# saiakarsh193/GenVox

Hardware: NVIDIA B200
Metric: Tacotron2 train mel-frames/s (higher is better)
Workload: dtype bf16

## Files before the change

genvox_b200/csrc/gvx_fused_bwd.cuh:

```cuda
#pragma once
#include <cooperative_groups.h>
#include <cuda_bf16.h>

#include "gvx_fused_fwd.cuh"

namespace gvx {

constexpr int FB_THREADS = 512;
constexpr int FB_NCOL = 48;
constexpr int FB_KSLAB = 16;
constexpr int FB_WSLAB_BYTES = FB_NCOL * 128;
constexpr int FB_RING = 8;
constexpr int FB_WLD_LD = 136;
constexpr int FB_QBYTES = FB_KSLAB * PC_CHUNK_BYTES;
constexpr int FB_PLD = 68;
constexpr int FB_DWQ = 5;

struct FbGeom {
    int RS, NH, NHP, nblk, NDS, nmt;
    __host__ __device__ FbGeom(int N, int RS_) {
        RS = RS_;
        NH = (((N + RS - 1) / RS) + 7) & ~7;
        NHP = (NH + 15) & ~15;
        nblk = NH / 8;
        NDS = NH + 40;
        nmt = NHP / 16;
    }
};

struct FbShared {
    uint64_t full[FB_RING], empty[FB_RING], tmem_full, wbar, thbar, xb[4];
    uint32_t tmem_slot;
    volatile int dead;
};

struct FbSmem {
    int ring, ths, dhqp, dqs, pdw, wsm, pin, cpart, dconvT, wlc, wldh, dctx, ctx32, w, de, dal, dwc, dcumc, v, xch, sh, total;
    __host__ __device__ FbSmem(int N, int RS) {
        const FbGeom g(N, RS);
        int o = 0;
        auto take = [&](int bytes) { int r = o; o += (bytes + 127) & ~127; return r; };
        ring = 0;
        ths = take(g.NHP * AF_D * 2);
        dqs = take(PC_ROWS * AF_D * 2);
        dhqp = take(4 * PC_ROWS * 8 * 4);
        pdw = take(16 * g.NHP * 4);
        o = o > FB_RING * PC_CHUNK_BYTES ? ((o + 1023) & ~1023) : FB_RING * PC_CHUNK_BYTES;
        wsm = take(FB_KSLAB * FB_WSLAB_BYTES);
        pin = take(4 * 12 * FB_PLD * 4);
        cpart = take(16 * 2 * g.NHP * 4);
        dconvT = take(AF_F * g.NDS * 4);
        wlc = take(AF_F * 2 * AF_KS * 4);
        wldh = take(AF_F * FB_WLD_LD * 2);
        dctx = take(FA_E * 4);
        ctx32 = take(FA_E * 4);
        w = take(g.NHP * 4);
        de = take(g.NHP * 4);
        dal = take(g.NHP * 4);
        dwc = take(g.NHP * 4);
        dcumc = take(g.NHP * 4);
        v = take(AF_D * 4);
        xch = take(64);
        sh = take((int)sizeof(FbShared));
        total = o + 1024;
    }
};

struct FbArgs {
    const __nv_bfloat16 *Wimg;
    uint8_t *gimg;
    const __nv_bfloat16 *WqB;
    const float *gates_stash;
    const float *c_stash;
    const float *dxdall;
    const float *dhc;
    int Kp, H;
    const float *d_align;
    const float *align;
    const float *ctx32;
    const __nv_bfloat16 *th;
    const __nv_bfloat16 *memb;
    const float *wlc, *wldT, *v;
    const int64_t *lengths;
    __nv_bfloat16 *dg_rm;
    __nv_bfloat16 *dq_rm;
    float *de_out;
    uint16_t *dconv_out;
    float *dctx_out;
    unsigned long long *dctxx;
    unsigned long long *dqx;
    unsigned *bar;
    int *err;
    DropCfg drop;
    int row_offset, B, N, T, RS;
    long long *dbg;
};

__device__ __forceinline__ void fb_gstamp(long long *dbg, int cta, int i, int k) {
    if (dbg && i == 20) dbg[32 * 1024 + cta * 16 + k] = fa_globaltimer();
}
__device__ __forceinline__ void fb_bar_w14() { asm volatile("bar.sync 2, 448;" ::: "memory"); }
__device__ __forceinline__ void st_async_f32(uint32_t caddr, float v, uint32_t cmbar) {
    asm volatile("st.async.weak.shared::cluster.mbarrier::complete_tx::bytes.f32 [%0], %1, [%2];" ::"r"(caddr), "f"(v), "r"(cmbar) : "memory");
}
__device__ __forceinline__ void st_async_f32x2(uint32_t caddr, float v0, float v1, uint32_t cmbar) {
    asm volatile("st.async.weak.shared::cluster.mbarrier::complete_tx::bytes.v2.f32 [%0], {%1, %2}, [%3];" ::"r"(caddr), "f"(v0), "f"(v1), "r"(cmbar)
                 : "memory");
}
__device__ __forceinline__ bool fb_wait_warp(uint64_t *bar, uint32_t parity, volatile int *dead, int *err, int code) {
    int ok = 1;
    if ((threadIdx.x & 31) == 0) ok = fa_wait_cluster(bar, parity, dead, err, code) ? 1 : 0;
    ok = __shfl_sync(0xffffffffu, ok, 0);
    if (ok) {
        while (!mbar_try_wait_cluster(bar, parity)) {}
    }
    return ok != 0;
}
__device__ __forceinline__ float4 fb_lstm_bwd_point(float dh_dropped, float mult, float4 ga, float c_prev, float c_new, float dc_in,
                                                    float &dc_prev) {
    const float dh = dh_dropped * mult;
    const float tc = tanh_fast(c_new);
    const float d_o = dh * tc;
    const float dc = dc_in + dh * ga.w * (1.f - tc * tc);
    const float d_i = dc * ga.z, d_g = dc * ga.x, d_f = dc * c_prev;
    dc_prev = dc * ga.y;
    return make_float4(d_i * ga.x * (1.f - ga.x), d_f * ga.y * (1.f - ga.y), d_g * (1.f - ga.z * ga.z), d_o * ga.w * (1.f - ga.w));
}

__global__ void __cluster_dims__(4, 1, 1) __launch_bounds__(FB_THREADS, 1) k_att_chain_bwd(const FbArgs a) {
    namespace cg = cooperative_groups;
    cg::cluster_group cluster = cg::this_cluster();
    extern __shared__ uint8_t smem_raw[];
    uint8_t *smem = smem_raw + ((1024u - (smem_u32(smem_raw) & 1023u)) & 1023u);
    const int N = a.N, T = a.T, B = a.B, RS = a.RS;
    const FbGeom G(N, RS);
    const FbSmem L(N, RS);
    uint8_t *ring = smem + L.ring, *wsm = smem + L.wsm, *ths = smem + L.ths;
    float *pin = (float *)(smem + L.pin), *cpart = (float *)(smem + L.cpart), *pdw = (float *)(smem + L.pdw);
    uint8_t *dqs = smem + L.dqs;
    float *dconvT = (float *)(smem + L.dconvT), *wlc = (float *)(smem + L.wlc);
    __nv_bfloat16 *wldh = (__nv_bfloat16 *)(smem + L.wldh);
    float *dctx = (float *)(smem + L.dctx), *ctx32 = (float *)(smem + L.ctx32);
    float *ws = (float *)(smem + L.w), *des = (float *)(smem + L.de), *dals = (float *)(smem + L.dal);
    float *dwc = (float *)(smem + L.dwc), *dcumc = (float *)(smem + L.dcumc), *vs = (float *)(smem + L.v);
    float *dhqp = (float *)(smem + L.dhqp);
    float *xch = (float *)(smem + L.xch);
    FbShared *sh = (FbShared *)(smem + L.sh);

    const int tid = threadIdx.x, wid = tid >> 5, lane = tid & 31, j = blockIdx.x;
    const int g4 = lane >> 2, tig = lane & 3;
    const int r = (int)cluster.block_rank(), c = j >> 2;
    const int row = RS == 2 ? 2 * c + (r >> 1) : c;
    const int prt = RS == 2 ? (r & 1) : r;
    const int gbase = RS == 2 ? (r & ~1) : 0;
    const bool rvalid = row < B;
    const int rowc = rvalid ? row : B - 1;
    const int len = a.lengths ? (int)a.lengths[rowc] : N;
    const int n_lo = prt * G.NH;
    const int n_own = rvalid ? max(0, min(N, n_lo + G.NH) - n_lo) : 0;
    const int own_len = max(0, min(len, n_lo + n_own) - n_lo);
    const bool th_live = n_own > 0;
    const bool has_left = prt > 0, has_right = prt < RS - 1;
    const int uk = tid & 7, ub = tid >> 3, uu = 8 * j + uk;
    const int ck = tid & 3, cb = (tid >> 2) & 63;
    const bool uvalid = ub < B;

    if (tid == 0) {
        for (int s = 0; s < FB_RING; ++s) { mbar_init(sh->full + s, 1); mbar_init(sh->empty + s, 1); }
        mbar_init(&sh->tmem_full, 1);
        mbar_init(&sh->wbar, 1);
        mbar_init(&sh->thbar, 1);
        for (int k = 0; k < 4; ++k) mbar_init(sh->xb + k, 1);
        sh->dead = 0;
        asm volatile("fence.mbarrier_init.release.cluster;" ::: "memory");
        asm volatile("fence.proxy.async.shared::cta;" ::: "memory");
    }
    if (wid == 0) {
        asm volatile("tcgen05.alloc.cta_group::1.sync.aligned.shared::cta.b32 [%0], %1;" ::"r"(smem_u32(&sh->tmem_slot)), "n"(64) : "memory");
        asm volatile("tcgen05.relinquish_alloc_permit.cta_group::1.sync.aligned;" ::: "memory");
    }
    for (int i = tid; i < AF_F * 2 * AF_KS; i += FB_THREADS) wlc[i] = a.wlc[i];
    for (int i = tid; i < AF_F * AF_D; i += FB_THREADS) wldh[(i >> 7) * FB_WLD_LD + (i & 127)] = __float2bfloat16(a.wldT[i]);
    if (tid < AF_D) vs[tid] = a.v[tid];
    for (int i = tid; i < AF_F * G.NDS; i += FB_THREADS) dconvT[i] = 0.f;
    for (int i = tid; i < G.NHP * AF_D / 2; i += FB_THREADS) reinterpret_cast<uint32_t *>(ths)[i] = 0u;
    for (int i = tid; i < G.NHP; i += FB_THREADS) { ws[i] = 0.f; des[i] = 0.f; dals[i] = 0.f; dwc[i] = 0.f; dcumc[i] = 0.f; }
    if (tid < 16) xch[tid] = 0.f;
    tc_fence_before();
    __syncthreads();
    tc_fence_after();
    const uint32_t tmem_base = sh->tmem_slot;
    if (tid == 0) {
        asm volatile("fence.proxy.async.shared::cta;" ::: "memory");
        mbar_expect_tx(&sh->wbar, FB_KSLAB * FB_WSLAB_BYTES);
        const uint8_t *wsrc = (const uint8_t *)a.Wimg + (size_t)j * FB_KSLAB * FB_WSLAB_BYTES;
        for (uint32_t off = 0; off < FB_KSLAB * FB_WSLAB_BYTES; off += 16384) tma_bulk_g2s(wsm + off, wsrc + off, 16384, &sh->wbar);
        if (th_live) {
            mbar_expect_tx(&sh->thbar, (uint32_t)n_own * AF_D * 2);
            tma_bulk_g2s(ths, a.th + (((size_t)(T - 1) * B + row) * N + n_lo) * AF_D, (uint32_t)n_own * AF_D * 2, &sh->thbar);
        }
    }
    const int qm = wid & 3, kq = wid >> 2;
    uint32_t wqf[2][2];
#pragma unroll
    for (int s = 0; s < 2; ++s)
#pragma unroll
        for (int hh = 0; hh < 2; ++hh) {
            const int d0 = 16 * (2 * kq + s) + 2 * tig + 8 * hh;
            const __nv_bfloat16 lo = a.WqB[(size_t)d0 * FA_A + 8 * j + g4], hi = a.WqB[(size_t)(d0 + 1) * FA_A + 8 * j + g4];
            wqf[s][hh] = (uint32_t)__bfloat16_as_ushort(lo) | ((uint32_t)__bfloat16_as_ushort(hi) << 16);
        }
    const uint32_t my_xch = smem_u32(xch), my_xb0 = smem_u32(sh->xb + 0), my_xb3 = smem_u32(sh->xb + 3), my_pin = smem_u32(pin);
    const uint32_t halo_bytes = (uint32_t)(min(AF_PAD, G.NH) * AF_F * 4) * (uint32_t)((has_left ? 1 : 0) + (has_right ? 1 : 0));
    const uint32_t my_dqs = smem_u32(dqs), my_xb1 = smem_u32(sh->xb + 1);
    const uint32_t nbl_dconv = mapa_u32(smem_u32(dconvT), (uint32_t)(gbase + max(prt - 1, 0)));
    const uint32_t nbr_dconv = mapa_u32(smem_u32(dconvT), (uint32_t)(gbase + min(prt + 1, RS - 1)));
    const uint32_t nbl_xb2 = mapa_u32(smem_u32(sh->xb + 2), (uint32_t)(gbase + max(prt - 1, 0)));
    const uint32_t nbr_xb2 = mapa_u32(smem_u32(sh->xb + 2), (uint32_t)(gbase + min(prt + 1, RS - 1)));

    DropCfg drop = a.drop;
    if (drop.kptr) { drop.k0 = drop.kptr[0]; drop.k1 = drop.kptr[1]; drop.kptr = nullptr; }
    float dc = 0.f, rec = 0.f;
    float c_new = uvalid ? a.c_stash[((size_t)T * B + ub) * FA_A + uu] : 0.f;
    const int quarter = j >> 5;
    const int kk0 = 4 * uu - 1024 * quarter;
    const size_t gimg_off = (size_t)quarter * FB_QBYTES + (size_t)(kk0 >> 6) * PC_CHUNK_BYTES + ub * 128 +
                            ((((kk0 & 63) >> 3) ^ (ub & 7)) << 4) + (kk0 & 7) * 2;
    unsigned *bq_own = a.bar + 16 * quarter + ((j & 31) >> 1);
    const unsigned *bq_need = a.bar + 16 * r;
    const size_t AE = FA_A + FA_E;

    if (tid < FA_E) {
        dctx[tid] = rvalid ? a.dhc[((size_t)(T - 1) * B + row) * a.Kp + a.H + tid] + a.dxdall[((size_t)(T - 1) * B + row) * AE + FA_A + tid] : 0.f;
        ctx32[tid] = rvalid ? a.ctx32[((size_t)(T - 1) * B + row) * FA_E + tid] : 0.f;
    }
    if (tid < G.NHP) {
        ws[tid] = tid < n_own ? a.align[((size_t)row * T + (T - 1)) * N + n_lo + tid] : 0.f;
        dals[tid] = (a.d_align && tid < n_own) ? a.d_align[((size_t)row * T + (T - 1)) * N + n_lo + tid] : 0.f;
    }
    if (wid == 0 && a.d_align && rvalid) {
        const float *al = a.align + ((size_t)row * T + (T - 1)) * N, *dal = a.d_align + ((size_t)row * T + (T - 1)) * N;
        for (int q = 0; q < RS; ++q) {
            const int q_lo = q * G.NH, q_own = max(0, min(N, q_lo + G.NH) - q_lo), q_len = max(0, min(len, q_lo + q_own) - q_lo);
            float p = 0.f;
            for (int n = lane; n < q_len; n += 32) p = fmaf(al[q_lo + n], dal[q_lo + n], p);
            p = warp_sum(p);
            if (lane == 0) xch[q] = p;
        }
    }
    __syncthreads();
    cluster.sync();
    const bool okw = fa_wait_mbar(&sh->wbar, 0, &sh->dead, a.err, 51);

    float mult = uvalid ? drop_mult(drop, SITE_ATT, (uint32_t)(T - 1), (uint32_t)(ub + a.row_offset), (uint32_t)uu) : 1.f;
    const __nv_bfloat16 *memb_b = a.memb + ((size_t)rowc * N + n_lo) * FA_E;
    uint4 mv[FB_DWQ][2];
    auto load_mem = [&](int mt0) {
#pragma unroll
        for (int q = 0; q < FB_DWQ; ++q) {
#pragma unroll
            for (int h2 = 0; h2 < 2; ++h2) {
                const int n = 16 * (mt0 + q) + g4 + 8 * h2;
                mv[q][h2] = n < own_len ? __ldg(reinterpret_cast<const uint4 *>(memb_b + (size_t)n * FA_E + 32 * wid + 8 * tig)) : make_uint4(0u, 0u, 0u, 0u);
            }
        }
    };
    load_mem(0);
    for (int i = 0; i < T; ++i) {
        const int t = T - 1 - i;
        const uint32_t par = (uint32_t)i & 1u;
        if (tid == 0) { pc_stamp(a.dbg, j, i, 0); fb_gstamp(a.dbg, j, i, 0); }
        if (i > 0 && tid < FA_E) {
            const unsigned long long *src = a.dctxx + ((size_t)par * PC_ROWS + rowc) * FA_E + tid;
            unsigned long long wv = 0ull;
            fa_spin([&] { wv = ld_relaxed_u64(src); return (unsigned)(wv >> 32) == (unsigned)i; }, &sh->dead, a.err, 52);
            if (rvalid) dctx[tid] += __uint_as_float((unsigned)wv);
        }
        if (tid < FA_E && rvalid && prt == 0) a.dctx_out[((size_t)t * B + row) * FA_E + tid] = dctx[tid];
        if (i > 0) fb_wait_warp(sh->xb + 0, par ^ 1u, &sh->dead, a.err, 53);
        if (th_live) fb_wait_warp(&sh->thbar, par, &sh->dead, a.err, 54);
        __syncthreads();
        if (tid == 0) {
            pc_stamp(a.dbg, j, i, 1);
            fb_gstamp(a.dbg, j, i, 1);
            mbar_expect_tx(sh->xb + 1, (uint32_t)PC_ROWS * AF_D * 2);
            if (halo_bytes) mbar_expect_tx(sh->xb + 2, halo_bytes);
            if (i + 1 < T) {
                mbar_expect_tx(sh->xb + 0, (uint32_t)RS * 4);
                mbar_expect_tx(sh->xb + 3, 4u * 12u * PC_ROWS * 4u);
            }
        }
        {
            uint32_t bfr[4] = {0u, 0u, 0u, 0u};
            if (g4 < 2) {
                const float4 d0 = *reinterpret_cast<const float4 *>(dctx + 32 * wid + 8 * tig), d1 = *reinterpret_cast<const float4 *>(dctx + 32 * wid + 8 * tig + 4);
                float x[8] = {d0.x, d0.y, d0.z, d0.w, d1.x, d1.y, d1.z, d1.w};
                if (g4 == 1) {
#pragma unroll
                    for (int k = 0; k < 8; ++k) x[k] -= __bfloat162float(__float2bfloat16(x[k]));
                }
#pragma unroll
                for (int k = 0; k < 4; ++k) bfr[k] = pack_bf2(x[2 * k], x[2 * k + 1]);
            }
            for (int mt0 = 0; mt0 < G.nmt; mt0 += FB_DWQ) {
                if (mt0 > 0) load_mem(mt0);
#pragma unroll
                for (int q = 0; q < FB_DWQ; ++q) {
                    if (mt0 + q < G.nmt) {
                        float acc[4] = {0.f, 0.f, 0.f, 0.f};
                        mma_bf16_16816(acc, mv[q][0].x, mv[q][1].x, mv[q][0].y, mv[q][1].y, bfr[0], bfr[1]);
                        mma_bf16_16816(acc, mv[q][0].z, mv[q][1].z, mv[q][0].w, mv[q][1].w, bfr[2], bfr[3]);
                        if (tig == 0) {
                            pdw[wid * G.NHP + 16 * (mt0 + q) + g4] = acc[0] + acc[1];
                            pdw[wid * G.NHP + 16 * (mt0 + q) + g4 + 8] = acc[2] + acc[3];
                        }
                    }
                }
            }
        }
        __syncthreads();
        if (tid == 0) pc_stamp(a.dbg, j, i, 12);
        if (wid * 32 < G.NHP) {
            float dot = 0.f;
#pragma unroll
            for (int h2 = 0; h2 < 2; ++h2) {
                const float4 g0 = *reinterpret_cast<const float4 *>(dctx + lane * 8 + 256 * h2), g1 = *reinterpret_cast<const float4 *>(dctx + lane * 8 + 256 * h2 + 4);
                const float4 c0 = *reinterpret_cast<const float4 *>(ctx32 + lane * 8 + 256 * h2), c1 = *reinterpret_cast<const float4 *>(ctx32 + lane * 8 + 256 * h2 + 4);
                dot = fmaf(c0.x, g0.x, dot); dot = fmaf(c0.y, g0.y, dot); dot = fmaf(c0.z, g0.z, dot); dot = fmaf(c0.w, g0.w, dot);
                dot = fmaf(c1.x, g1.x, dot); dot = fmaf(c1.y, g1.y, dot); dot = fmaf(c1.z, g1.z, dot); dot = fmaf(c1.w, g1.w, dot);
            }
            dot = warp_sum(dot);
            for (int p = 0; p < RS; ++p) dot += xch[p];
            const int n = tid;
            if (n < G.NHP) {
                float dwn = 0.f;
#pragma unroll
                for (int w8 = 0; w8 < 16; ++w8) dwn += pdw[w8 * G.NHP + n];
                dwn += (dwc[n] + dcumc[n]) + dals[n];
                const float de = n < own_len ? ws[n] * (dwn - dot) : 0.f;
                des[n] = de;
                if (n < n_own) a.de_out[((size_t)t * B + row) * N + n_lo + n] = de;
            }
        }
        __syncthreads();
        if (tid == 0) pc_stamp(a.dbg, j, i, 13);
        {
            const float4 va = *reinterpret_cast<const float4 *>(vs + 8 * wid), vb = *reinterpret_cast<const float4 *>(vs + 8 * wid + 4);
            const float vv[8] = {va.x, va.y, va.z, va.w, vb.x, vb.y, vb.z, vb.w};
            float acc[8];
#pragma unroll
            for (int k = 0; k < 8; ++k) acc[k] = 0.f;
            for (int n = lane; n < G.NHP; n += 32) {
                uint4 *tp = reinterpret_cast<uint4 *>(ths + n * 256 + ((wid ^ (n & 7)) << 4));
                const float de = des[n];
                const uint4 tw = *tp;
                const float th[8] = {bf_lo(tw.x), bf_hi(tw.x), bf_lo(tw.y), bf_hi(tw.y), bf_lo(tw.z), bf_hi(tw.z), bf_lo(tw.w), bf_hi(tw.w)};
                float sv[8];
#pragma unroll
                for (int k = 0; k < 8; ++k) {
                    sv[k] = n < own_len ? de * vv[k] * (1.f - th[k] * th[k]) : 0.f;
                    acc[k] += sv[k];
                }
                *tp = make_uint4(pack_bf2(sv[0], sv[1]), pack_bf2(sv[2], sv[3]), pack_bf2(sv[4], sv[5]), pack_bf2(sv[6], sv[7]));
            }
#pragma unroll
            for (int o = 16; o > 0; o >>= 1) {
#pragma unroll
                for (int k = 0; k < 8; ++k) acc[k] += __shfl_xor_sync(0xffffffffu, acc[k], o);
            }
            if (lane < 4) {
                const float q0 = lane == 0 ? acc[0] : (lane == 1 ? acc[2] : (lane == 2 ? acc[4] : acc[6]));
                const float q1 = lane == 0 ? acc[1] : (lane == 1 ? acc[3] : (lane == 2 ? acc[5] : acc[7]));
                const int d2 = 4 * wid + lane;
                if (rvalid)
                    st_relaxed_u64(a.dqx + (((size_t)par * PC_ROWS + row) * 4 + prt) * (AF_D / 2) + d2,
                                   ((unsigned long long)(unsigned)(i + 1) << 32) | pack_bf2(q0, q1));
            }
        }
        if (tid == 0) { pc_stamp(a.dbg, j, i, 2); fb_gstamp(a.dbg, j, i, 2); }
        float4 ga = make_float4(0.f, 0.f, 0.f, 0.f);
        float c_prev = 0.f, dxd = 0.f;
        if (uvalid) {
            ga = __ldcs(reinterpret_cast<const float4 *>(a.gates_stash + ((size_t)t * B + ub) * 4 * FA_A + 4 * uu));
            c_prev = __ldcs(a.c_stash + ((size_t)t * B + ub) * FA_A + uu);
            dxd = __ldcs(a.dxdall + ((size_t)t * B + ub) * AE + uu);
        }
        if (tid == 0) pc_stamp(a.dbg, j, i, 14);
        for (int task = wid; task < 2 * G.nmt; task += 16) {
            const int mt = task >> 1, nh = task & 1;
            const int n0 = 16 * mt + g4, n1 = n0 + 8;
            const uint8_t *tr0 = ths + n0 * 256 + 4 * tig, *tr1 = ths + n1 * 256 + 4 * tig;
            const int sw0 = n0 & 7, sw1 = n1 & 7;
            float acc[2][4] = {{0.f, 0.f, 0.f, 0.f}, {0.f, 0.f, 0.f, 0.f}};
            const __nv_bfloat16 *bh = wldh + (16 * nh + g4) * FB_WLD_LD + 2 * tig;
#pragma unroll
            for (int s = 0; s < 8; ++s) {
                const int ch = 2 * s;
                const uint32_t a0 = *reinterpret_cast<const uint32_t *>(tr0 + ((ch ^ sw0) << 4));
                const uint32_t a1 = *reinterpret_cast<const uint32_t *>(tr1 + ((ch ^ sw1) << 4));
                const uint32_t a2 = *reinterpret_cast<const uint32_t *>(tr0 + (((ch + 1) ^ sw0) << 4));
                const uint32_t a3 = *reinterpret_cast<const uint32_t *>(tr1 + (((ch + 1) ^ sw1) << 4));
#pragma unroll
                for (int nt = 0; nt < 2; ++nt) {
                    const uint32_t b0 = *reinterpret_cast<const uint32_t *>(bh + 8 * nt * FB_WLD_LD + 16 * s);
                    const uint32_t b1 = *reinterpret_cast<const uint32_t *>(bh + 8 * nt * FB_WLD_LD + 16 * s + 8);
                    mma_bf16_16816(acc[nt], a0, a1, a2, a3, b0, b1);
                }
            }
#pragma unroll
            for (int nt = 0; nt < 2; ++nt) {
                const int f0 = 16 * nh + 8 * nt + 2 * tig;
#pragma unroll
                for (int hr = 0; hr < 2; ++hr) {
                    const int n = hr == 0 ? n0 : n1;
                    const float x0 = acc[nt][2 * hr], x1 = acc[nt][2 * hr + 1];
                    if (n < G.NH) {
                        dconvT[f0 * G.NDS + AF_PAD + n] = x0;
                        dconvT[(f0 + 1) * G.NDS + AF_PAD + n] = x1;
                        if (n < n_own) *reinterpret_cast<uint32_t *>(a.dconv_out + (((size_t)t * B + row) * N + n_lo + n) * AF_F + f0) = pack_bf2(x0, x1);
                        if (has_left && n < AF_PAD) {
                            st_async_f32(nbl_dconv + 4 * (f0 * G.NDS + AF_PAD + G.NH + n), x0, nbl_xb2);
                            st_async_f32(nbl_dconv + 4 * ((f0 + 1) * G.NDS + AF_PAD + G.NH + n), x1, nbl_xb2);
                        }
                        if (has_right && n >= G.NH - AF_PAD) {
                            st_async_f32(nbr_dconv + 4 * (f0 * G.NDS + n - (G.NH - AF_PAD)), x0, nbr_xb2);
                            st_async_f32(nbr_dconv + 4 * ((f0 + 1) * G.NDS + n - (G.NH - AF_PAD)), x1, nbr_xb2);
                        }
                    }
                }
            }
        }
        if (tid == 0) pc_stamp(a.dbg, j, i, 15);
        __syncthreads();
        if (tid == 0) { pc_stamp(a.dbg, j, i, 3); fb_gstamp(a.dbg, j, i, 3); }

        {
            const int grow = 16 * r + (tid >> 5);
            const unsigned long long *qsrc = a.dqx + ((size_t)par * PC_ROWS + grow) * 4 * (AF_D / 2) + 2 * lane;
            float q4[4] = {0.f, 0.f, 0.f, 0.f};
            if (grow < B) {
                unsigned long long wv[4][2];
                fa_spin([&] {
                    bool all = true;
#pragma unroll
                    for (int p = 0; p < 4; ++p) {
                        if (p < RS) {
#pragma unroll
                            for (int k = 0; k < 2; ++k) {
                                wv[p][k] = ld_relaxed_u64(qsrc + (size_t)p * (AF_D / 2) + k);
                                all = all && (unsigned)(wv[p][k] >> 32) == (unsigned)(i + 1);
                            }
                        }
                    }
                    return all;
                }, &sh->dead, a.err, 57);
#pragma unroll
                for (int p = 0; p < 4; ++p) {
                    if (p < RS) {
#pragma unroll
                        for (int k = 0; k < 2; ++k) {
                            q4[2 * k] += bf_lo((uint32_t)wv[p][k]);
                            q4[2 * k + 1] += bf_hi((uint32_t)wv[p][k]);
                        }
                    }
                }
            }
            const uint32_t w0 = pack_bf2(q4[0], q4[1]), w1 = pack_bf2(q4[2], q4[3]);
            if (grow < B) *reinterpret_cast<uint2 *>(a.dq_rm + ((size_t)t * B + grow) * AF_D + 4 * lane) = make_uint2(w0, w1);
            const uint32_t doff = (uint32_t)(grow * 256 + (((lane >> 1) ^ (grow & 7)) << 4) + (lane & 1) * 8);
#pragma unroll
            for (int p = 0; p < 4; ++p)
                st_async_f32x2(mapa_u32(my_dqs + doff, (uint32_t)p), __uint_as_float(w0), __uint_as_float(w1), mapa_u32(my_xb1, (uint32_t)p));
            fb_wait_warp(sh->xb + 1, par, &sh->dead, a.err, 55);
            const int rA = 16 * qm + g4, rB = rA + 8;
            const uint8_t *ra = dqs + rA * 256 + 4 * tig, *rb = dqs + rB * 256 + 4 * tig;
            float cf[4] = {0.f, 0.f, 0.f, 0.f};
#pragma unroll
            for (int s2 = 0; s2 < 2; ++s2) {
                const int ch = 2 * (2 * kq + s2);
                const uint32_t a0 = *reinterpret_cast<const uint32_t *>(ra + ((ch ^ (rA & 7)) << 4));
                const uint32_t a1 = *reinterpret_cast<const uint32_t *>(rb + ((ch ^ (rB & 7)) << 4));
                const uint32_t a2 = *reinterpret_cast<const uint32_t *>(ra + (((ch + 1) ^ (rA & 7)) << 4));
                const uint32_t a3 = *reinterpret_cast<const uint32_t *>(rb + (((ch + 1) ^ (rB & 7)) << 4));
                mma_bf16_16816(cf, a0, a1, a2, a3, wqf[s2][0], wqf[s2][1]);
            }
            *reinterpret_cast<float2 *>(dhqp + ((size_t)(kq * PC_ROWS + rA)) * 8 + 2 * tig) = make_float2(cf[0], cf[1]);
            *reinterpret_cast<float2 *>(dhqp + ((size_t)(kq * PC_ROWS + rB)) * 8 + 2 * tig) = make_float2(cf[2], cf[3]);
        }
        __syncthreads();
        if (tid == 0) { pc_stamp(a.dbg, j, i, 4); fb_gstamp(a.dbg, j, i, 4); }
        {
            uint2 dgp = make_uint2(0u, 0u);
            if (uvalid) {
                const float dhq = ((dhqp[(0 * PC_ROWS + ub) * 8 + uk] + dhqp[(1 * PC_ROWS + ub) * 8 + uk]) + dhqp[(2 * PC_ROWS + ub) * 8 + uk]) +
                                  dhqp[(3 * PC_ROWS + ub) * 8 + uk];
                const float dh = dhq + dxd + rec;
                float dcp;
                const float4 d4 = fb_lstm_bwd_point(dh, mult, ga, c_prev, c_new, dc, dcp);
                dc = dcp;
                c_new = c_prev;
                dgp = make_uint2(pack_bf2(d4.x, d4.y), pack_bf2(d4.z, d4.w));
                *reinterpret_cast<uint2 *>(a.gimg + (size_t)par * 4 * FB_QBYTES + gimg_off) = dgp;
                fence_proxy_async_global();
            }
            __syncthreads();
            if (tid == 0) { gbar_arrive(bq_own); pc_stamp(a.dbg, j, i, 5); fb_gstamp(a.dbg, j, i, 5); }
            if (uvalid) *reinterpret_cast<uint2 *>(a.dg_rm + ((size_t)t * B + ub) * 4 * FA_A + 4 * uu) = dgp;
        }
        if (i + 1 == T) break;

        if (tid < FA_E) {
            dctx[tid] = rvalid ? __ldcs(a.dhc + ((size_t)(t - 1) * B + row) * a.Kp + a.H + tid) + __ldcs(a.dxdall + ((size_t)(t - 1) * B + row) * AE + FA_A + tid) : 0.f;
            ctx32[tid] = rvalid ? __ldcs(a.ctx32 + ((size_t)(t - 1) * B + row) * FA_E + tid) : 0.f;
        }
        if (tid < G.NHP) {
            ws[tid] = tid < n_own ? a.align[((size_t)row * T + (t - 1)) * N + n_lo + tid] : 0.f;
            if (a.d_align) dals[tid] = tid < n_own ? a.d_align[((size_t)row * T + (t - 1)) * N + n_lo + tid] : 0.f;
        }
        if (wid == 0) {
            if (elect_one()) {
                const unsigned target = 2u * (unsigned)(i + 1);
                const uint8_t *src = a.gimg + (size_t)par * 4 * FB_QBYTES + (size_t)r * FB_QBYTES;
                uint32_t pending = okw ? 0xffffu : 0u, have = 0u;
                bool first = true;
                const long long t0 = clock64();
                while (pending) {
                    unsigned cnt[16];
#pragma unroll
                    for (int q4 = 0; q4 < 3; ++q4)
                        asm volatile("ld.relaxed.gpu.global.v4.u32 {%0,%1,%2,%3}, [%4];"
                                     : "=r"(cnt[4 * q4]), "=r"(cnt[4 * q4 + 1]), "=r"(cnt[4 * q4 + 2]), "=r"(cnt[4 * q4 + 3])
                                     : "l"(bq_need + 4 * q4)
                                     : "memory");
                    asm volatile("ld.acquire.gpu.global.v4.u32 {%0,%1,%2,%3}, [%4];"
                                 : "=r"(cnt[12]), "=r"(cnt[13]), "=r"(cnt[14]), "=r"(cnt[15])
                                 : "l"(bq_need + 12)
                                 : "memory");
                    uint32_t ready = 0;
#pragma unroll
                    for (int s = 0; s < 16; ++s)
                        if (cnt[s] >= target) ready |= 1u << s;
                    ready &= pending;
                    if (ready) {
                        fence_proxy_async_global();
                        if (first) {
                            pc_stamp(a.dbg, j, i, 8);
                            fb_gstamp(a.dbg, j, i, 8);
                            asm volatile("fence.proxy.async.shared::cta;" ::: "memory");
                            first = false;
                        }
#pragma unroll 1
                        for (int s = 0; s < 8; ++s) {
                            if (!(ready >> s & 1u)) continue;
                            mbar_expect_tx(sh->full + s, PC_CHUNK_BYTES);
                            tma_bulk_g2s(ring + (size_t)s * PC_CHUNK_BYTES, src + (size_t)s * PC_CHUNK_BYTES, PC_CHUNK_BYTES, sh->full + s);
                        }
                        pending &= ~(ready & 0xffu);
                        have |= ready;
                    }
                    if ((pending & 0xffu) == 0u && (have & 0xff00u) == 0xff00u) break;
                    if (sh->dead) break;
                    if (clock64() - t0 > FA_WAIT_CYCLES) { sh->dead = 1; atomicCAS(a.err, 0, 58); break; }
                }
                if (!sh->dead && (have & 0xff00u) == 0xff00u) {
#pragma unroll 1
                    for (int s = 8; s < 16; ++s) {
                        const int slot = s - 8;
                        if (!fa_wait_mbar(sh->empty + slot, 0u, &sh->dead, a.err, 59)) break;
                        mbar_expect_tx(sh->full + slot, PC_CHUNK_BYTES);
                        tma_bulk_g2s(ring + (size_t)slot * PC_CHUNK_BYTES, src + (size_t)s * PC_CHUNK_BYTES, PC_CHUNK_BYTES, sh->full + slot);
                    }
                }
                pc_stamp(a.dbg, j, i, 9);
            }
            __syncwarp();
        } else if (wid == 1) {
            if (elect_one()) {
                constexpr uint32_t idesc = umma_idesc_bf16(64, FB_NCOL);
                const uint64_t a0 = umma_desc_sw128(smem_u32(ring)), b0 = umma_desc_sw128(smem_u32(wsm));
                bool ok = okw;
                static_assert(FB_KSLAB == 16, "the issue loop below is unrolled for two revolutions of the 8-slot ring");
#pragma unroll
                for (int s = 0; s < FB_KSLAB; ++s) {
                    const int ring_slot = s & 7;
                    if (ok && !mbar_try_wait(sh->full + ring_slot, (uint32_t)(s >> 3))) ok = fa_wait_mbar(sh->full + ring_slot, (uint32_t)(s >> 3), &sh->dead, a.err, 60);
                    if (s == 0) pc_stamp(a.dbg, j, i, 10);
                    if (ok) {
                        tc_fence_after();
                        const uint64_t ad = a0 + (uint64_t)(ring_slot * (PC_CHUNK_BYTES >> 4)), bd = b0 + (uint64_t)(s * (FB_WSLAB_BYTES >> 4));
                        umma_bf16(tmem_base, ad, bd, idesc, s > 0 ? 1u : 0u);
                        umma_bf16(tmem_base, ad + 2, bd + 2, idesc, 1u);
                        umma_bf16(tmem_base, ad + 4, bd + 4, idesc, 1u);
                        umma_bf16(tmem_base, ad + 6, bd + 6, idesc, 1u);
                        umma_commit(sh->empty + ring_slot);
                    }
                }
                if (ok) umma_commit(&sh->tmem_full);
                pc_stamp(a.dbg, j, i, 11);
                fa_wait_mbar(&sh->tmem_full, par, &sh->dead, a.err, 61);
            }
            __syncwarp();
        } else {
            const int wt = tid - 64;
            if (has_left || has_right) fb_wait_warp(sh->xb + 2, par, &sh->dead, a.err, 56);
            {
                const int ntask = 16 * 2 * G.nblk;
                for (int task = wt; task < ntask; task += 448) {
                    const int fp = task & 15, rest = task >> 4;
                    const int ch = rest / G.nblk, m0 = (rest - ch * G.nblk) * 8;
                    float acc[8];
#pragma unroll
                    for (int q = 0; q < 8; ++q) acc[q] = 0.f;
#pragma unroll
                    for (int ff = 0; ff < 2; ++ff) {
                        const int f = 2 * fp + ff;
                        float x[40];
                        const float4 *xr = reinterpret_cast<const float4 *>(dconvT + f * G.NDS + m0);
#pragma unroll
                        for (int q = 0; q < 10; ++q) {
                            const float4 t4 = xr[q];
                            x[4 * q] = t4.x; x[4 * q + 1] = t4.y; x[4 * q + 2] = t4.z; x[4 * q + 3] = t4.w;
                        }
                        const float *wr = wlc + (f * 2 + ch) * AF_KS;
#pragma unroll
                        for (int k = 0; k < AF_KS; ++k) {
                            const float wk = wr[k];
#pragma unroll
                            for (int q = 0; q < 8; ++q) acc[q] = fmaf(wk, x[q - k + 30], acc[q]);
                        }
                    }
                    float4 *dst = reinterpret_cast<float4 *>(cpart + (fp * 2 + ch) * G.NH + m0);
                    dst[0] = make_float4(acc[0], acc[1], acc[2], acc[3]);
                    dst[1] = make_float4(acc[4], acc[5], acc[6], acc[7]);
                }
            }
            fb_bar_w14();
            if (wt < 2 * G.NH) {
                const int ch = wt >= G.NH, m = wt - ch * G.NH;
                float s = 0.f;
#pragma unroll
                for (int fp = 0; fp < 16; ++fp) s += cpart[(fp * 2 + ch) * G.NH + m];
                if (ch == 0) dwc[m] = s;
                else dcumc[m] += s;
            }
            fb_bar_w14();
            if (wid == 2) {
                float p = 0.f;
                for (int n = lane; n < own_len; n += 32) p = fmaf(ws[n], (dwc[n] + dcumc[n]) + dals[n], p);
                p = warp_sum(p);
                if (lane < RS) st_async_f32(mapa_u32(my_xch + 4 * prt, (uint32_t)(gbase + lane)), p, mapa_u32(my_xb0, (uint32_t)(gbase + lane)));
            }
        }
        load_mem(0);
        if (uvalid) mult = drop_mult(drop, SITE_ATT, (uint32_t)(t - 1), (uint32_t)(ub + a.row_offset), (uint32_t)uu);
        __syncthreads();
        const bool okt = sh->dead == 0;
        if (tid == 0) { pc_stamp(a.dbg, j, i, 6); fb_gstamp(a.dbg, j, i, 6); }
        if (wid == 0 && elect_one()) {
            if (th_live) {
                mbar_expect_tx(&sh->thbar, (uint32_t)n_own * AF_D * 2);
                tma_bulk_g2s(ths, a.th + (((size_t)(t - 1) * B + row) * N + n_lo) * AF_D, (uint32_t)n_own * AF_D * 2, &sh->thbar);
            }
        }
        if (wid >= 4 && okt) {
            const int q = wid & 3, cg3 = (wid >> 2) - 1;
            float vals[16];
            tc_fence_after();
            tmem_ld16(tmem_base + ((uint32_t)(32 * q) << 16) + (uint32_t)(16 * cg3), vals);
            tc_fence_before();
            if (lane < 16) {
                const int b = 16 * q + lane;
#pragma unroll
                for (int n = 0; n < 16; ++n) {
                    const int col = 16 * cg3 + n;
                    const int owner = col < 32 ? col >> 3 : (col - 32) >> 2;
                    const int off = (r * 12 + (col < 32 ? col & 7 : 8 + ((col - 32) & 3))) * FB_PLD + b;
                    st_async_f32(mapa_u32(my_pin + 4 * off, (uint32_t)owner), vals[n], mapa_u32(my_xb3, (uint32_t)owner));
                }
            }
        }
        fb_wait_warp(sh->xb + 3, par, &sh->dead, a.err, 62);
        {
            const int o = uk * FB_PLD + ub;
            rec = ((pin[o] + pin[12 * FB_PLD + o]) + pin[24 * FB_PLD + o]) + pin[36 * FB_PLD + o];
            if (tid < 256) {
                const float *cp4 = pin + (8 + ck) * FB_PLD + cb;
                const float cx = ((cp4[0] + cp4[12 * FB_PLD]) + cp4[24 * FB_PLD]) + cp4[36 * FB_PLD];
                if (cb < B)
                    st_relaxed_u64(a.dctxx + ((size_t)(par ^ 1u) * PC_ROWS + cb) * FA_E + 4 * j + ck,
                                   ((unsigned long long)(unsigned)(i + 1) << 32) | (unsigned long long)__float_as_uint(cx));
            }
        }
        if (tid == 0) { pc_stamp(a.dbg, j, i, 7); fb_gstamp(a.dbg, j, i, 7); }
    }
    __syncthreads();
    cluster.sync();
    if (wid == 0) {
        asm volatile("tcgen05.dealloc.cta_group::1.sync.aligned.b32 %0, %1;" ::"r"(tmem_base), "n"(64) : "memory");
    }
}

__global__ void k_fb_pack_w(const float *__restrict__ Wa_packed, int Ka, int P, __nv_bfloat16 *__restrict__ img) {
    const size_t per_cta = (size_t)FB_KSLAB * FB_NCOL * 64, total = 128 * per_cta;
    for (size_t i = (size_t)blockIdx.x * blockDim.x + threadIdx.x; i < total; i += (size_t)gridDim.x * blockDim.x) {
        const int j = (int)(i / per_cta);
        const int rem = (int)(i - (size_t)j * per_cta);
        const int slab = rem / (FB_NCOL * 64), rr = rem - slab * FB_NCOL * 64;
        const int n = rr >> 6, cpos = (rr >> 3) & 7, e = rr & 7;
        const int kk = slab * 64 + ((cpos ^ (n & 7)) << 3) + e;
        const int cc = j >> 2, rk = j & 3;
        const int grow = 1024 * rk + kk;
        const int col = n < 32 ? P + FA_E + 32 * cc + n : P + 16 * cc + (n - 32);
        img[i] = __float2bfloat16(Wa_packed[(size_t)grow * Ka + col]);
    }
}
inline size_t fb_wimg_elems() { return (size_t)128 * FB_KSLAB * FB_NCOL * 64; }
inline size_t fb_gimg_bytes() { return (size_t)2 * 4 * FB_QBYTES; }
inline size_t fb_dctxx_words() { return (size_t)2 * PC_ROWS * FA_E; }
inline size_t fb_dqx_words() { return (size_t)2 * PC_ROWS * 4 * (AF_D / 2); }

inline int fb_row_split(int B, int N) { return (B <= 32 && FbGeom(N, 4).NH >= 16) ? 4 : 2; }

inline bool fb_supported(const Dims &d, int B, int N) {
    static int sms = -1;
    if (sms < 0) {
        int dev = 0;
        cudaGetDevice(&dev);
        cudaDeviceGetAttribute(&sms, cudaDevAttrMultiProcessorCount, dev);
    }
    if (d.A != FA_A || d.E != FA_E || d.D != AF_D || d.F != AF_F || d.KS != AF_KS) return false;
    if (B < 1 || B > PC_ROWS || N < 1 || sms < 128 || d.P % 8 != 0 || d.H % 8 != 0) return false;
    const int RS = fb_row_split(B, N);
    if (FbGeom(N, RS).NH > ((FA_MAXN / 2 + 7) & ~7)) return false;
    const size_t smem = FbSmem(N, RS).total;
    if (smem > 227 * 1024) return false;
    static size_t cached_smem = 0;
    static bool cached = false;
    if (cached_smem != smem) {
        cached = 4 * max_resident_clusters(k_att_chain_bwd, FB_THREADS, smem, 4, 128) >= 128;
        cached_smem = smem;
    }
    return cached;
}

inline int launch_att_chain_bwd(const FbArgs &a_in, cudaStream_t st) {
    FbArgs a = a_in;
    a.dbg = pc_dbg_buffer() ? pc_dbg_buffer() + 32 * 1024 : nullptr;
    const size_t smem = FbSmem(a.N, a.RS).total;
    static size_t configured = 0;
    if (configured < smem) {
        GVX_CUDA(cudaFuncSetAttribute(k_att_chain_bwd, cudaFuncAttributeMaxDynamicSharedMemorySize, (int)smem));
        configured = smem;
    }
    GVX_CUDA(cudaMemsetAsync(a.bar, 0, 64 * sizeof(unsigned), st));
    GVX_CUDA(cudaMemsetAsync(a.dctxx, 0, fb_dctxx_words() * sizeof(unsigned long long), st));
    GVX_CUDA(cudaMemsetAsync(a.dqx, 0, fb_dqx_words() * sizeof(unsigned long long), st));
    GVX_CUDA(cudaMemsetAsync(a.gimg, 0, fb_gimg_bytes(), st));
    k_att_chain_bwd<<<128, FB_THREADS, smem, st>>>(a);
    GVX_LAUNCHED(1);
    GVX_CUDA(cudaGetLastError());
    return 0;
}

}
```

profiles/bwd_chain_timeline.py:

```python
import os
import sys

import numpy as np
import torch

ROOT = os.path.dirname(os.path.dirname(os.path.abspath(__file__)))
sys.path.insert(0, ROOT)
sys.path.insert(0, os.path.join(ROOT, "tests"))
import genvox_b200
from genvox_b200 import _native
from oracle import synth
from test_cuda_parity import make_decoder

B, N, T = (int(x) for x in sys.argv[1:4]) if len(sys.argv) >= 4 else (64, 150, 48)
lib = _native.load()
dev = torch.device("cuda:0")
dims = synth.DecoderDims()
W = synth.make_decoder_weights(23, dims)
mem, mel, lens = synth.make_inputs(67, B, N, T, dims, ragged=False)
dec = make_decoder(dims, W, dev, True)
dec.precision = "bf16"
dbg = torch.zeros(4, 1024, 32, dtype=torch.int64, device=dev)
x_mem, x_mel, x_len = torch.from_numpy(mem).to(dev), torch.from_numpy(mel).to(dev), torch.from_numpy(lens).to(dev)


def step():
    dec.zero_grad(set_to_none=True)
    m, g, a = dec(x_mem.clone().requires_grad_(True), x_mel, x_len)
    (m.sum() + g.sum()).backward()
    torch.cuda.synchronize()
    genvox_b200.check_device_errors()


step()
lib.gvx_debug_timeline(dbg.data_ptr())
step()
lib.gvx_debug_timeline(None)
x = dbg[1, :T].cpu().numpy().astype(np.float64)
names = ["iter start", "d ctx assembled (poll, carry dots, tanh tile)", "d w / d e / d q partial published", "d conv mma + halo push done",
         "d q rows arrived, d h_q", "d gates written, barrier arrive", "tmem_full (TMA + MMA; conv transpose overlapped)",
         "partials pushed + summed, d ctx published"]
per = np.diff(x[2:-1, 0])
print(f"B={B} N={N} T={T}: iteration period median {np.median(per):.0f} cyc = {np.median(per) / 1.965e3:.2f} us (p10 {np.percentile(per, 10):.0f}, p90 {np.percentile(per, 90):.0f})")
for k, n in ((12, "  (d w partials on mma, sync)"), (13, "  (d e written, sync)"), (14, "  (cell inputs requested)"), (15, "  (warp 0: its d conv tile done)"), (8, "  (TMA: image barrier passed)"),
             (10, "  (MMA: first slab landed)"), (9, "  (TMA: last slab issued)"), (11, "  (MMA: last slab issued)")):
    print(f"    {n:46s} +{np.median(x[2:-1, k] - x[2:-1, 0]):7.0f} cyc")
prev = 0.0
for i, n in enumerate(names):
    d = np.median(x[2:-1, i] - x[2:-1, 0])
    print(f"  {i} {n:48s} +{d:7.0f} cyc  ({(d - prev) / 1.965e3:5.2f} us)")
    prev = d

g = dbg[2].reshape(-1)[: 128 * 16].cpu().numpy().astype(np.float64).reshape(128, 16)
ev = {0: "iter start", 1: "d ctx assembled", 2: "d q published", 3: "d conv done", 4: "d q rows arrived", 5: "image barrier arrive",
      8: "image barrier passed", 6: "tmem_full", 7: "d ctx published"}
t0 = g[:, 0].min()
print("per-CTA event times at iteration 20, ns after the first CTA started it: min / median / max (argmax CTA)")
for k in (0, 1, 2, 3, 4, 5, 8, 6, 7):
    col = g[:, k] - t0
    print(f"  {ev[k]:24s} {col.min():8.0f} {np.median(col):8.0f} {col.max():8.0f}   (CTA {int(col.argmax())}; CTA 0: {col[0]:.0f})")
```

Before: 1.398 million.

## Move conv-transpose carry dot before dq wait and copy image slabs per-warp with cp.async

The conv-transpose reduction, carry dot and next-step input loads now run on all warps earlier in the iteration, before the dq-row wait, rather than on 14 warps overlapped with the image fetch. The single-thread polling loop that issued TMA bulk copies for 16 slabs is replaced by each of the 16 warps polling its own counter and copying its slab with cp.async, then arriving on the full mbarrier. The generic-to-async proxy fence after writing gates is dropped. The aim is to shorten the serialized critical path by spreading polling and copying across warps, at the cost of losing the previous overlap of conv work with the TMA wait and of more threads spinning on global counters.

Measured after the change: 1.258 million, median of 6. 0.899x the previous value.

```diff
diff --git a/genvox_b200/csrc/gvx_fused_bwd.cuh b/genvox_b200/csrc/gvx_fused_bwd.cuh
--- a/genvox_b200/csrc/gvx_fused_bwd.cuh
+++ b/genvox_b200/csrc/gvx_fused_bwd.cuh
@@ -99,7 +99,11 @@
 __device__ __forceinline__ void fb_gstamp(long long *dbg, int cta, int i, int k) {
     if (dbg && i == 20) dbg[32 * 1024 + cta * 16 + k] = fa_globaltimer();
 }
-__device__ __forceinline__ void fb_bar_w14() { asm volatile("bar.sync 2, 448;" ::: "memory"); }
+__device__ __forceinline__ unsigned fb_ld_relaxed_u32(const unsigned *p) {
+    unsigned v;
+    asm volatile("ld.relaxed.gpu.global.u32 %0, [%1];" : "=r"(v) : "l"(p) : "memory");
+    return v;
+}
 __device__ __forceinline__ void st_async_f32(uint32_t caddr, float v, uint32_t cmbar) {
     asm volatile("st.async.weak.shared::cluster.mbarrier::complete_tx::bytes.f32 [%0], %1, [%2];" ::"r"(caddr), "f"(v), "r"(cmbar) : "memory");
 }
@@ -434,6 +438,69 @@
         __syncthreads();
         if (tid == 0) { pc_stamp(a.dbg, j, i, 3); fb_gstamp(a.dbg, j, i, 3); }
 
+        float cdot = 0.f;
+        if (i + 1 < T) {
+            float dctx_n = 0.f, ctx_n = 0.f, w_n = 0.f, dal_n = 0.f;
+            if (tid < FA_E && rvalid) {
+                dctx_n = __ldcs(a.dhc + ((size_t)(t - 1) * B + row) * a.Kp + a.H + tid) + __ldcs(a.dxdall + ((size_t)(t - 1) * B + row) * AE + FA_A + tid);
+                ctx_n = __ldcs(a.ctx32 + ((size_t)(t - 1) * B + row) * FA_E + tid);
+            }
+            if (tid < n_own) {
+                w_n = a.align[((size_t)row * T + (t - 1)) * N + n_lo + tid];
+                if (a.d_align) dal_n = a.d_align[((size_t)row * T + (t - 1)) * N + n_lo + tid];
+            }
+            if (has_left || has_right) fb_wait_warp(sh->xb + 2, par, &sh->dead, a.err, 56);
+            {
+                const int ntask = 16 * 2 * G.nblk;
+                for (int task = tid; task < ntask; task += FB_THREADS) {
+                    const int fp = task & 15, rest = task >> 4;
+                    const int ch = rest / G.nblk, m0 = (rest - ch * G.nblk) * 8;
+                    float acc[8];
+#pragma unroll
+                    for (int q = 0; q < 8; ++q) acc[q] = 0.f;
+#pragma unroll
+                    for (int ff = 0; ff < 2; ++ff) {
+                        const int f = 2 * fp + ff;
+                        float x[40];
+                        const float4 *xr = reinterpret_cast<const float4 *>(dconvT + f * G.NDS + m0);
+#pragma unroll
+                        for (int q = 0; q < 10; ++q) {
+                            const float4 t4 = xr[q];
+                            x[4 * q] = t4.x; x[4 * q + 1] = t4.y; x[4 * q + 2] = t4.z; x[4 * q + 3] = t4.w;
+                        }
+                        const float *wr = wlc + (f * 2 + ch) * AF_KS;
+#pragma unroll
+                        for (int k = 0; k < AF_KS; ++k) {
+                            const float wk = wr[k];
+#pragma unroll
+                            for (int q = 0; q < 8; ++q) acc[q] = fmaf(wk, x[q - k + 30], acc[q]);
+                        }
+                    }
+                    float4 *dst = reinterpret_cast<float4 *>(cpart + (fp * 2 + ch) * G.NH + m0);
+                    dst[0] = make_float4(acc[0], acc[1], acc[2], acc[3]);
+                    dst[1] = make_float4(acc[4], acc[5], acc[6], acc[7]);
+                }
+            }
+            __syncthreads();
+            if (tid < FA_E) { dctx[tid] = dctx_n; ctx32[tid] = ctx_n; }
+            if (tid < G.NHP) { ws[tid] = w_n; dals[tid] = dal_n; }
+            if (tid < 2 * G.NH) {
+                const int ch = tid >= G.NH, m = tid - ch * G.NH;
+                float s = 0.f;
+#pragma unroll
+                for (int fp = 0; fp < 16; ++fp) s += cpart[(fp * 2 + ch) * G.NH + m];
+                if (ch == 0) dwc[m] = s;
+                else dcumc[m] += s;
+            }
+            __syncthreads();
+            if (wid == 2) {
+                float p = 0.f;
+                for (int n = lane; n < own_len; n += 32) p = fmaf(ws[n], (dwc[n] + dcumc[n]) + dals[n], p);
+                cdot = warp_sum(p);
+            }
+            if (tid == 0) pc_stamp(a.dbg, j, i, 16);
+        }
+
         {
             const int grow = 16 * r + (tid >> 5);
             const unsigned long long *qsrc = a.dqx + ((size_t)par * PC_ROWS + grow) * 4 * (AF_D / 2) + 2 * lane;
@@ -472,6 +539,8 @@
             for (int p = 0; p < 4; ++p)
                 st_async_f32x2(mapa_u32(my_dqs + doff, (uint32_t)p), __uint_as_float(w0), __uint_as_float(w1), mapa_u32(my_xb1, (uint32_t)p));
             fb_wait_warp(sh->xb + 1, par, &sh->dead, a.err, 55);
+            if (wid == 2 && i + 1 < T && lane < RS)
+                st_async_f32(mapa_u32(my_xch + 4 * prt, (uint32_t)(gbase + lane)), cdot, mapa_u32(my_xb0, (uint32_t)(gbase + lane)));
             const int rA = 16 * qm + g4, rB = rA + 8;
             const uint8_t *ra = dqs + rA * 256 + 4 * tig, *rb = dqs + rB * 256 + 4 * tig;
             float cf[4] = {0.f, 0.f, 0.f, 0.f};
@@ -501,7 +570,6 @@
                 c_new = c_prev;
                 dgp = make_uint2(pack_bf2(d4.x, d4.y), pack_bf2(d4.z, d4.w));
                 *reinterpret_cast<uint2 *>(a.gimg + (size_t)par * 4 * FB_QBYTES + gimg_off) = dgp;
-                fence_proxy_async_global();
             }
             __syncthreads();
             if (tid == 0) { gbar_arrive(bq_own); pc_stamp(a.dbg, j, i, 5); fb_gstamp(a.dbg, j, i, 5); }
@@ -509,72 +577,28 @@
         }
         if (i + 1 == T) break;
 
-        if (tid < FA_E) {
-            dctx[tid] = rvalid ? __ldcs(a.dhc + ((size_t)(t - 1) * B + row) * a.Kp + a.H + tid) + __ldcs(a.dxdall + ((size_t)(t - 1) * B + row) * AE + FA_A + tid) : 0.f;
-            ctx32[tid] = rvalid ? __ldcs(a.ctx32 + ((size_t)(t - 1) * B + row) * FA_E + tid) : 0.f;
-        }
-        if (tid < G.NHP) {
-            ws[tid] = tid < n_own ? a.align[((size_t)row * T + (t - 1)) * N + n_lo + tid] : 0.f;
-            if (a.d_align) dals[tid] = tid < n_own ? a.d_align[((size_t)row * T + (t - 1)) * N + n_lo + tid] : 0.f;
-        }
-        if (wid == 0) {
-            if (elect_one()) {
-                const unsigned target = 2u * (unsigned)(i + 1);
-                const uint8_t *src = a.gimg + (size_t)par * 4 * FB_QBYTES + (size_t)r * FB_QBYTES;
-                uint32_t pending = okw ? 0xffffu : 0u, have = 0u;
-                bool first = true;
-                const long long t0 = clock64();
-                while (pending) {
-                    unsigned cnt[16];
-#pragma unroll
-                    for (int q4 = 0; q4 < 3; ++q4)
-                        asm volatile("ld.relaxed.gpu.global.v4.u32 {%0,%1,%2,%3}, [%4];"
-                                     : "=r"(cnt[4 * q4]), "=r"(cnt[4 * q4 + 1]), "=r"(cnt[4 * q4 + 2]), "=r"(cnt[4 * q4 + 3])
-                                     : "l"(bq_need + 4 * q4)
-                                     : "memory");
-                    asm volatile("ld.acquire.gpu.global.v4.u32 {%0,%1,%2,%3}, [%4];"
-                                 : "=r"(cnt[12]), "=r"(cnt[13]), "=r"(cnt[14]), "=r"(cnt[15])
-                                 : "l"(bq_need + 12)
-                                 : "memory");
-                    uint32_t ready = 0;
-#pragma unroll
-                    for (int s = 0; s < 16; ++s)
-                        if (cnt[s] >= target) ready |= 1u << s;
-                    ready &= pending;
-                    if (ready) {
-                        fence_proxy_async_global();
-                        if (first) {
-                            pc_stamp(a.dbg, j, i, 8);
-                            fb_gstamp(a.dbg, j, i, 8);
-                            asm volatile("fence.proxy.async.shared::cta;" ::: "memory");
-                            first = false;
-                        }
-#pragma unroll 1
-                        for (int s = 0; s < 8; ++s) {
-                            if (!(ready >> s & 1u)) continue;
-                            mbar_expect_tx(sh->full + s, PC_CHUNK_BYTES);
-                            tma_bulk_g2s(ring + (size_t)s * PC_CHUNK_BYTES, src + (size_t)s * PC_CHUNK_BYTES, PC_CHUNK_BYTES, sh->full + s);
-                        }
-                        pending &= ~(ready & 0xffu);
-                        have |= ready;
-                    }
-                    if ((pending & 0xffu) == 0u && (have & 0xff00u) == 0xff00u) break;
-                    if (sh->dead) break;
-                    if (clock64() - t0 > FA_WAIT_CYCLES) { sh->dead = 1; atomicCAS(a.err, 0, 58); break; }
-                }
-                if (!sh->dead && (have & 0xff00u) == 0xff00u) {
-#pragma unroll 1
-                    for (int s = 8; s < 16; ++s) {
-                        const int slot = s - 8;
-                        if (!fa_wait_mbar(sh->empty + slot, 0u, &sh->dead, a.err, 59)) break;
-                        mbar_expect_tx(sh->full + slot, PC_CHUNK_BYTES);
-                        tma_bulk_g2s(ring + (size_t)slot * PC_CHUNK_BYTES, src + (size_t)s * PC_CHUNK_BYTES, PC_CHUNK_BYTES, sh->full + slot);
-                    }
-                }
-                pc_stamp(a.dbg, j, i, 9);
-            }
-            __syncwarp();
-        } else if (wid == 1) {
+        {
+            const int slot = wid & 7;
+            const unsigned target = 2u * (unsigned)(i + 1);
+            const unsigned *ctr = bq_need + wid;
+            bool ok = okw && fa_spin([&] { return fb_ld_relaxed_u32(ctr) >= target; }, &sh->dead, a.err, 58);
+            ok = __all_sync(0xffffffffu, ok && ld_acquire_u32(ctr) >= target) != 0;
+            if (tid == 0) { pc_stamp(a.dbg, j, i, 8); fb_gstamp(a.dbg, j, i, 8); }
+            if (wid >= 8 && ok) ok = fb_wait_warp(sh->empty + slot, 0u, &sh->dead, a.err, 59);
+            if (ok) {
+                const uint8_t *src = a.gimg + (size_t)par * 4 * FB_QBYTES + (size_t)r * FB_QBYTES + (size_t)wid * PC_CHUNK_BYTES;
+                uint8_t *dst = ring + (size_t)slot * PC_CHUNK_BYTES;
+#pragma unroll
+                for (int v = lane; v < PC_CHUNK_BYTES / 16; v += 32) cp_async16(dst + 16 * v, src + 16 * v, true);
+                cp_async_commit();
+                cp_async_wait<0>();
+                asm volatile("fence.proxy.async.shared::cta;" ::: "memory");
+                __syncwarp();
+                if (lane == 0) asm volatile("mbarrier.arrive.shared::cta.b64 _, [%0];" ::"r"(smem_u32(sh->full + slot)) : "memory");
+            }
+            if (wid == 15 && lane == 0) pc_stamp(a.dbg, j, i, 9);
+        }
+        if (wid == 1) {
             if (elect_one()) {
                 constexpr uint32_t idesc = umma_idesc_bf16(64, FB_NCOL);
                 const uint64_t a0 = umma_desc_sw128(smem_u32(ring)), b0 = umma_desc_sw128(smem_u32(wsm));
@@ -600,56 +624,6 @@
                 fa_wait_mbar(&sh->tmem_full, par, &sh->dead, a.err, 61);
             }
             __syncwarp();
-        } else {
-            const int wt = tid - 64;
-            if (has_left || has_right) fb_wait_warp(sh->xb + 2, par, &sh->dead, a.err, 56);
-            {
-                const int ntask = 16 * 2 * G.nblk;
-                for (int task = wt; task < ntask; task += 448) {
-                    const int fp = task & 15, rest = task >> 4;
-                    const int ch = rest / G.nblk, m0 = (rest - ch * G.nblk) * 8;
-                    float acc[8];
-#pragma unroll
-                    for (int q = 0; q < 8; ++q) acc[q] = 0.f;
-#pragma unroll
-                    for (int ff = 0; ff < 2; ++ff) {
-                        const int f = 2 * fp + ff;
-                        float x[40];
-                        const float4 *xr = reinterpret_cast<const float4 *>(dconvT + f * G.NDS + m0);
-#pragma unroll
-                        for (int q = 0; q < 10; ++q) {
-                            const float4 t4 = xr[q];
-                            x[4 * q] = t4.x; x[4 * q + 1] = t4.y; x[4 * q + 2] = t4.z; x[4 * q + 3] = t4.w;
-                        }
-                        const float *wr = wlc + (f * 2 + ch) * AF_KS;
-#pragma unroll
-                        for (int k = 0; k < AF_KS; ++k) {
-                            const float wk = wr[k];
-#pragma unroll
-                            for (int q = 0; q < 8; ++q) acc[q] = fmaf(wk, x[q - k + 30], acc[q]);
-                        }
-                    }
-                    float4 *dst = reinterpret_cast<float4 *>(cpart + (fp * 2 + ch) * G.NH + m0);
-                    dst[0] = make_float4(acc[0], acc[1], acc[2], acc[3]);
-                    dst[1] = make_float4(acc[4], acc[5], acc[6], acc[7]);
-                }
-            }
-            fb_bar_w14();
-            if (wt < 2 * G.NH) {
-                const int ch = wt >= G.NH, m = wt - ch * G.NH;
-                float s = 0.f;
-#pragma unroll
-                for (int fp = 0; fp < 16; ++fp) s += cpart[(fp * 2 + ch) * G.NH + m];
-                if (ch == 0) dwc[m] = s;
-                else dcumc[m] += s;
-            }
-            fb_bar_w14();
-            if (wid == 2) {
-                float p = 0.f;
-                for (int n = lane; n < own_len; n += 32) p = fmaf(ws[n], (dwc[n] + dcumc[n]) + dals[n], p);
-                p = warp_sum(p);
-                if (lane < RS) st_async_f32(mapa_u32(my_xch + 4 * prt, (uint32_t)(gbase + lane)), p, mapa_u32(my_xb0, (uint32_t)(gbase + lane)));
-            }
         }
         load_mem(0);
         if (uvalid) mult = drop_mult(drop, SITE_ATT, (uint32_t)(t - 1), (uint32_t)(ub + a.row_offset), (uint32_t)uu);
diff --git a/profiles/bwd_chain_timeline.py b/profiles/bwd_chain_timeline.py
--- a/profiles/bwd_chain_timeline.py
+++ b/profiles/bwd_chain_timeline.py
@@ -38,12 +38,13 @@
 lib.gvx_debug_timeline(None)
 x = dbg[1, :T].cpu().numpy().astype(np.float64)
 names = ["iter start", "d ctx assembled (poll, carry dots, tanh tile)", "d w / d e / d q partial published", "d conv mma + halo push done",
-         "d q rows arrived, d h_q", "d gates written, barrier arrive", "tmem_full (TMA + MMA; conv transpose overlapped)",
+         "d q rows arrived, d h_q", "d gates written, barrier arrive", "tmem_full (image copy + MMA)",
          "partials pushed + summed, d ctx published"]
 per = np.diff(x[2:-1, 0])
 print(f"B={B} N={N} T={T}: iteration period median {np.median(per):.0f} cyc = {np.median(per) / 1.965e3:.2f} us (p10 {np.percentile(per, 10):.0f}, p90 {np.percentile(per, 90):.0f})")
-for k, n in ((12, "  (d w partials on mma, sync)"), (13, "  (d e written, sync)"), (14, "  (cell inputs requested)"), (15, "  (warp 0: its d conv tile done)"), (8, "  (TMA: image barrier passed)"),
-             (10, "  (MMA: first slab landed)"), (9, "  (TMA: last slab issued)"), (11, "  (MMA: last slab issued)")):
+for k, n in ((12, "  (d w partials on mma, sync)"), (13, "  (d e written, sync)"), (14, "  (cell inputs requested)"), (15, "  (warp 0: its d conv tile done)"),
+             (16, "  (conv transpose + carry dot done)"), (8, "  (warp 0: slab 0 counter acquired)"), (10, "  (MMA: first slab landed)"),
+             (9, "  (warp 15: last slab landed)"), (11, "  (MMA: last slab issued)")):
     print(f"    {n:46s} +{np.median(x[2:-1, k] - x[2:-1, 0]):7.0f} cyc")
 prev = 0.0
 for i, n in enumerate(names):
@@ -53,7 +54,7 @@
 
 g = dbg[2].reshape(-1)[: 128 * 16].cpu().numpy().astype(np.float64).reshape(128, 16)
 ev = {0: "iter start", 1: "d ctx assembled", 2: "d q published", 3: "d conv done", 4: "d q rows arrived", 5: "image barrier arrive",
-      8: "image barrier passed", 6: "tmem_full", 7: "d ctx published"}
+      8: "slab 0 counter acquired", 6: "tmem_full", 7: "d ctx published"}
 t0 = g[:, 0].min()
 print("per-CTA event times at iteration 20, ns after the first CTA started it: min / median / max (argmax CTA)")
 for k in (0, 1, 2, 3, 4, 5, 8, 6, 7):
```
